# maniacs-ops/ringpop-go

Measured on AMD Instinct MI355X. Metric: simulated member-rounds/sec at 64k members, higher is better.
Workload: dtype u32; 1 GPU; config3_cascade: 65536 members, 655 killed at r=10; rounds 5-592 timed (steady state, kill, suspect wave; faulty wave from r>=35 in window); members=65536, live_member_rounds=38153303, parallelism=1 GPU

## Files before the change

### include/swimsim.h

```cpp
#ifndef SWIMSIM_H
#define SWIMSIM_H
#include <stddef.h>
#include <stdint.h>

#ifdef __cplusplus
extern "C" {
#endif

#define SWIMSIM_ABI_VERSION 12

enum {
    SWIMSIM_OK = 0,
    SWIMSIM_EINVAL = -1,
    SWIMSIM_ENOMEM = -2,
    SWIMSIM_EHIP = -3,
    SWIMSIM_ECAPACITY = -4,
    SWIMSIM_ERANGE = -5
};

enum { SWIMSIM_ALIVE = 0, SWIMSIM_SUSPECT = 1, SWIMSIM_FAULTY = 2, SWIMSIM_LEAVE = 3, SWIMSIM_TOMBSTONE = 4,
       SWIMSIM_UNKNOWN = 7 };
#define SWIMSIM_SOURCE_NONE (-1)

typedef struct swimsim_config {
// ... 14 lines not shown
    uint64_t message_pool_bytes;
    uint32_t observer_begin, observer_end;
    const struct swimsim_tuning *tuning;
} swimsim_config;

typedef struct swimsim_tuning {
    int32_t hot_slots;
    int32_t dense_slots;
    int32_t cs_async;
    int32_t cs_async_rows;
    int32_t cs_narrow_rows;
    int32_t cs_ref;
    int32_t fault_inject;
    int32_t defer_test;
    int32_t cs_defer;
} swimsim_tuning;

enum {
    SWIMSIM_EV_KILL = 1,
    SWIMSIM_EV_REVIVE = 2,
    SWIMSIM_EV_REINCARNATE = 3,
    SWIMSIM_EV_LEAVE = 4,
    SWIMSIM_EV_PARTITION = 5,
    SWIMSIM_EV_HEAL = 6,
    SWIMSIM_EV_REAP = 7,
    SWIMSIM_EV_CLOCK = 8
};
typedef struct swimsim_event { uint32_t round; uint32_t kind; int32_t a; int32_t b; } swimsim_event;

enum {
// ... 126 lines not shown
```

### ringpop-go_amd/csrc/swimsim_device.h

```cpp
#pragma once
#include <hip/hip_runtime.h>
#include <stdint.h>

namespace swimdev {

constexpr uint32_t ST_ALIVE = 0, ST_SUSPECT = 1, ST_FAULTY = 2, ST_LEAVE = 3, ST_TOMB = 4, ST_UNKNOWN = 7;
constexpr uint32_t SRC_NONE = 0xFFFFFFFFu;
constexpr uint32_t NO_DEADLINE = 0xFFFFFFFFu;
constexpr uint8_t DP_NONE = 0xFF;
constexpr uint32_t DE_NONE = 0xFFFFFFFFu;
__host__ __device__ inline uint32_t de_p(uint32_t x) { return x >> 24; }
__host__ __device__ inline uint32_t de_src(uint32_t x) { return (x & 0xFFFFFFu) == 0xFFFFFFu ? SRC_NONE : (x & 0xFFFFFFu); }
__host__ __device__ inline uint32_t de_x(uint32_t src, uint32_t p) { return (src & 0xFFFFFFu) | (p << 24); }

enum Counter {
    C_ROUNDS, C_PINGS, C_PINGS_OK, C_PINGREQS, C_HELPER_CALLS, C_HELPER_ERRORS, C_INCONCLUSIVE,
    C_SUSPECT_DECL, C_APPLIED, C_REFUTES, C_FULL_SYNCS, C_FULL_SYNCS_PINGREQ, C_RFS_DONE, C_RFS_OMITTED,
    C_TIMERS_FIRED, C_MSG_CHANGES, C_HEAL_ATTEMPTS, C_HEAL_FAILURES, C_NCOUNTERS,
    C_X_MERGED = C_NCOUNTERS, C_X_APPLIED, C_X_ISSUED, C_X_CS_ROWS, C_X_CS_DUP,
    C_X_MERGED_R, C_X_APPLIED_R, C_X_RISSUED, C_X_RCALLS, C_X_BUMPED, C_X_CS_ROWS_N, C_X_CSD_SCANNED,
    C_X_DENSE_RESP, C_X_DENSE_JOBS, C_X_JOBS_APPLIED, C_X_DENSE_HEAL,
    C_X_DEFER, C_X_DEFER_EQ, C_X_DEFER_NOROW, C_X_DEFER_REP, C_X_DEFER_UNDO,
    C_X_DEFER_REP_DIFF, C_X_DEFER_UNDO_DIFF, C_X_DEFER_FS, C_X_DEFER_UNDO_OVER, C_X_DEFER_CLEAN,
    C_X_ISSUE_SNAPS, C_X_LAZY_LATE, C_X_LAZY_MAT, C_NALL
};

constexpr int CTR_SHARDS = 64, CTR_STRIDE = 64;
static_assert(C_NALL <= CTR_STRIDE, "counter block too small");
constexpr uint32_t POOL_SHARDS = 64, POOL_CUR_STRIDE = 16;

enum ErrBits : uint32_t {
    E_POOL = 1, E_DENSE = 2, E_ECAP = 4, E_SHORT = 8, E_ITER = 16, E_COUNT = 32, E_XCAP = 64
};

struct MsgDesc {
    uint32_t off_lo, off_hi;
    uint32_t len;
    uint32_t kind;
};
// ... 58 lines not shown
    uint32_t *hmw;
    uint2 *hde;
    uint32_t *colx;
    uint32_t *hotnew;
    uint32_t *hot_cnt;
    uint32_t HP;
    int32_t *nhe;
    uint32_t *ucl, *uhk, *ucold, *ucnt;
    uint2 *ulog;
    uint32_t *ulog_cnt;
    uint32_t ulog_cap;
    uint32_t ulog_stride;
    uint32_t defer_test;
    uint32_t *ilen;
    int32_t *ilast;
};
constexpr uint32_t ULOG_CAP = 1024, ULOG_STRIDE = ULOG_CAP + 256;
constexpr uint32_t SRC_PEND = 0x7FFFFFFEu, SRC_CLAIM = 0x7FFFFFFDu;
constexpr uint32_t DIRTY_CARRIED = 2u;

__device__ __forceinline__ uint32_t hot_slot(const DS &d, uint32_t m) { return d.hidx ? d.hidx[m] : SRC_NONE; }

__host__ __device__ inline bool is_pingable(uint32_t st) { return st <= ST_SUSPECT; }

__device__ __forceinline__ uint32_t clock_of(const DS &d, uint32_t o, uint32_t r) { return r + (uint32_t)d.coff[o]; }

constexpr uint32_t RT_LOOKUP = 0, RT_COLD = 8191, RT_MAXSLOTS = 8128;
__host__ __device__ inline uint32_t rec_m(const uint4 &r) { return r.x & 0xFFFFFFu; }
__host__ __device__ inline uint32_t rec_st(const uint4 &r) { return (r.x >> 24) & 7u; }
__host__ __device__ inline uint32_t rec_e(const uint4 &r) { return r.y & 0xFFFFFFu; }
__host__ __device__ inline uint32_t rec_tag(const uint4 &r) { return (r.x >> 27) | ((r.y >> 24) << 5); }
__host__ __device__ inline uint32_t tag_of_slot(uint32_t hk) { return hk == SRC_NONE ? RT_COLD : hk + 1u; }
__host__ __device__ inline uint4 rec_make(uint32_t m, uint32_t st, uint32_t e, uint32_t src, uint32_t sinc, uint32_t tag) {
    return make_uint4(m | (st << 24) | (tag << 27), e | ((tag >> 5) << 24), src, sinc);
}
__host__ __device__ inline uint4 rec_retag(const uint4 &r, uint32_t tag) {
    return make_uint4((r.x & 0x07FFFFFFu) | (tag << 27), (r.y & 0xFFFFFFu) | ((tag >> 5) << 24), r.z, r.w);
}
__device__ __forceinline__ uint32_t rec_slot(const DS &d, const uint4 &r) {
    const uint32_t t = rec_tag(r);
    return t == RT_LOOKUP ? hot_slot(d, rec_m(r)) : t == RT_COLD ? SRC_NONE : t - 1u;
}
// ... 138 lines not shown
```

### ringpop-go_amd/csrc/swimsim_engine.hip

```cpp
#include "swimsim_kernels.hip"
#include "swimsim_xchg.hip"
#include "swimsim_census.hip"
#include "swimsim_route.hip"

#include <hipcub/hipcub.hpp>
#include <rccl/rccl.h>

#include <algorithm>
#include <cmath>
#include <condition_variable>
#include <cstdarg>
#include <cstdio>
#include <cstring>
#include <memory>
#include <mutex>
#include <string>
#include <thread>
#include <vector>

#include "../../include/swimsim.h"

using namespace swimdev;

namespace {
// ... 333 lines not shown
    size_t rt_bytes_cap = 0, rt_keys_cap = 0, rt_rows_cap = 0, rt_own_cap = 0, rt_exc_cap = 0, rt_cub_bytes = 0;
    std::vector<uint64_t> rt_rel;
    hipEvent_t rt_ev[2] = {nullptr, nullptr};
    int csr_mode = 1;
    CsrSet csr, csr2;
    size_t csr_sbw_words = 0;
    uint32_t csr_ecap = 4096, csr_rcap = 1024, csr_KP = 0;
    uint64_t csr_launches = 0;
    uint32_t csr_side_min = 4097;
    int fault_inject = 0;
    int defer_test = 0;
    int cs_defer = 1;
    uint32_t rounds_left = 0;
    uint32_t round_deferred = 0;
    bool cs_carried = false;
    bool cs_defer_log = false;
    uint64_t cs_skipped_rounds = 0, cs_carried_rows = 0, cs_forced = 0, cs_units_base[3] = {0, 0, 0};
    bool colx_stale = false;
    std::string err;

    int fail(int code, const char *fmt, ...) {
        char buf[512];
        va_list ap;
        va_start(ap, fmt);
        vsnprintf(buf, sizeof buf, fmt, ap);
        va_end(ap);
        err = buf;
        return code;
    }
};
// ... 1259 lines not shown
        return bail(SWIMSIM_EHIP);
    }
    const swimsim_tuning *tun = cfg->tuning;
    if (tun && tun->cs_async >= 0) h->cs_async = tun->cs_async != 0;
    if (tun && tun->cs_narrow_rows >= 0) h->cs_narrow_rows = (uint32_t)tun->cs_narrow_rows;
    if (tun && tun->cs_ref >= 0) h->csr_mode = tun->cs_ref;
    if (tun && tun->fault_inject > 0) h->fault_inject = tun->fault_inject;
    if (tun && tun->defer_test > 0) h->defer_test = tun->defer_test;
    if (tun && tun->cs_defer >= 0) h->cs_defer = tun->cs_defer;
    if (const char *v = getenv("SWIMSIM_CS_DEFER")) h->cs_defer = atoi(v);
    if (const char *v = getenv("SWIMSIM_CS_DEFER_LOG")) h->cs_defer_log = atoi(v) != 0;
    if (h->cs_defer < 0 || h->cs_defer > 2) {
        h->err = "swimsim_tuning.cs_defer is -1, 0, 1 or 2";
        return bail(SWIMSIM_EINVAL);
    }
    if (h->fault_inject & 32) h->csr_ecap = 24;
    if (h->fault_inject & 256) h->csr_side_min = 1024;
    if (const char *v = getenv("SWIMSIM_SYNC_SPIN")) h->sync_spin = atoi(v) != 0;
    if (const char *v = getenv("SWIMSIM_SIDE2"))
        if (atoi(v) == 0 && h->side2) { hipStreamDestroy(h->side2); h->side2 = nullptr; }
    DS &d = h->d;
    d.N = h->N; d.NP = h->NP; d.NL = h->NL; d.lo = h->lo;
    d.NB = h->NP / 64;
    d.NBW = (d.NB + 63) / 64;
    d.NBIT = ((h->NP / 32) + 3) & ~3u;
    d.W = h->W; d.pfactor = h->pfactor; d.K = h->K; d.maxjobs = h->maxjobs;
    d.to_susp = h->to_susp; d.to_faulty = h->to_faulty; d.to_tomb = h->to_tomb;
    d.seed = h->seed;
    const size_t rows = (size_t)h->NL * h->NP;
    int rc = 0;
// ... 14 lines not shown
        (rc = dalloc(h, &d.colx, d.NBIT, "divergent columns")) || (rc = dalloc(h, &d.ucl, h->N, "divergent column list")) ||
        (rc = dalloc(h, &d.uhk, h->N, "divergent column hot slots")) || (rc = dalloc(h, &d.ucold, h->N, "cold divergent columns")) ||
        (rc = dalloc(h, &d.ucnt, 2, "divergent column counts")))
        return bail(rc);
    hipMemset(d.nhe, 0, (size_t)h->NL * 4);
    hipMemset(d.coff, 0, (size_t)h->N * 4);
    h->coff.assign(h->N, 0);
    hipMemset(d.colx, 0xFF, (size_t)d.NBIT * 4);
    hipMemset(d.cpslot, 0xFF, (size_t)h->NL * 4);
    {
        uint32_t hp = std::min<uint32_t>(2048u, h->NP);
        if (tun && tun->hot_slots >= 0) hp = std::min<uint32_t>((uint32_t)tun->hot_slots, h->NP);
        hp = std::min<uint32_t>((hp + 63) & ~63u, RT_MAXSLOTS);
        d.hidx = nullptr; d.hlist = nullptr; d.hmw = nullptr; d.hde = nullptr; d.hotnew = nullptr; d.hot_cnt = nullptr;
        d.HP = 0;
        if (hp) {
            if ((rc = dalloc(h, &d.hidx, h->N, "hot index")) || (rc = dalloc(h, &d.hlist, hp, "hot list")) ||
                (rc = dalloc(h, &d.hmw, (size_t)h->NL * hp, "hot member words")) ||
                (rc = dalloc(h, &d.hde, (size_t)h->NL * hp, "hot dissemination cells")) ||
                (rc = dalloc(h, &d.hotnew, d.NBIT, "hot candidates")) || (rc = dalloc(h, &d.hot_cnt, 2, "hot count")))
                return bail(rc);
            d.HP = hp;
            hot_reset(h, false);
        }
    }
    {
        std::vector<uint32_t> aw((size_t)h->N * 6, 0u);
        for (uint32_t m = 0; m < h->N; m++) {
            uint8_t b[24] = {0};
            memcpy(b, h->addrs[m].data(), h->W);
            for (int w = 0; w < 6; w++)
                aw[(size_t)m * 6 + w] = (uint32_t)b[4 * w] | ((uint32_t)b[4 * w + 1] << 8) | ((uint32_t)b[4 * w + 2] << 16) |
                                        ((uint32_t)b[4 * w + 3] << 24);
        }
        uint32_t *dev = nullptr;
        if ((rc = dalloc(h, &dev, aw.size(), "address words"))) return bail(rc);
        if (hipMemcpy(dev, aw.data(), aw.size() * 4, hipMemcpyHostToDevice) != hipSuccess) return bail(SWIMSIM_EHIP);
// ... 1067 lines not shown
        }
    }
    if (n) *n = F_NFAM;
    return SWIMSIM_OK;
}

int swimsim_kernel_units(swimsim_t *h, const char **names, double *values, size_t cap, size_t *n) {
    if (!h) return SWIMSIM_EINVAL;
    uint64_t c[CTR_STRIDE];
    if (int rc = read_counters(h, c)) return rc;
    static const char *kn[] = {"cs_rows_wide", "cs_rows_narrow", "cs_dup_rows", "recv_merged", "recv_applied",
                               "recv_issued", "recv_calls", "resp_merged", "resp_applied", "resp_bumped", "issued",
                               "bitmap_words_per_row", "hot_slots", "dense_resp", "dense_jobs", "jobs_applied",
                               "dense_heal", "defer", "defer_eq", "defer_norow", "defer_rep", "defer_undo",
                               "defer_rep_diff", "defer_undo_diff", "defer_fs", "defer_undo_over", "defer_clean",
                               "issue_snaps", "lazy_late", "lazy_mat",
                               "cs_skipped_rounds", "cs_carried_rows", "cs_forced"};
    const int ki[] = {C_X_CS_ROWS, C_X_CS_ROWS_N, C_X_CS_DUP, C_X_MERGED, C_X_APPLIED, C_X_RISSUED, C_X_RCALLS,
                      C_X_MERGED_R, C_X_APPLIED_R, C_X_BUMPED, C_X_ISSUED, -1, -2, C_X_DENSE_RESP, C_X_DENSE_JOBS,
                      C_X_JOBS_APPLIED, C_X_DENSE_HEAL, C_X_DEFER, C_X_DEFER_EQ, C_X_DEFER_NOROW, C_X_DEFER_REP,
                      C_X_DEFER_UNDO, C_X_DEFER_REP_DIFF, C_X_DEFER_UNDO_DIFF, C_X_DEFER_FS, C_X_DEFER_UNDO_OVER,
                      C_X_DEFER_CLEAN, C_X_ISSUE_SNAPS, C_X_LAZY_LATE, C_X_LAZY_MAT,
                      -3, -4, -5};
    const uint64_t lazy_c[3] = {h->cs_skipped_rounds - h->cs_units_base[0], h->cs_carried_rows - h->cs_units_base[1],
                                h->cs_forced - h->cs_units_base[2]};
    static_assert(sizeof(kn) / sizeof(kn[0]) == sizeof(ki) / sizeof(ki[0]), "one counter per name");
    uint32_t hot = 0;
    if (h->d.hot_cnt) {
        HIPCHK(h, hipMemcpyAsync(&hot, h->d.hot_cnt, 4, hipMemcpyDeviceToHost, h->s));
        HIPCHK(h, stream_sync(h));
    }
    const size_t k = sizeof(ki) / sizeof(ki[0]);
    for (size_t i = 0; i < k && i < cap; i++) {
        if (names) names[i] = kn[i];
        if (values)
            values[i] = ki[i] == -1 ? (double)h->d.NBIT : ki[i] == -2 ? (double)hot : ki[i] <= -3 ? (double)lazy_c[-3 - ki[i]]
                                                                                : (double)(c[ki[i]] - h->fam_bytes_base[ki[i]]);
// ... 197 lines not shown
```

### ringpop-go_amd/csrc/swimsim_kernels.hip

```cpp
#include "swimsim_kernels.h"

namespace swimdev {

#define SWIM_DPP(old, src, ctrl, rm) ((uint32_t)__builtin_amdgcn_update_dpp((int)(old), (int)(src), (ctrl), (rm), 0xf, false))
template <typename Op>
__device__ __forceinline__ uint32_t dpp_scan(uint32_t x, uint32_t id, Op op) {
    x = op(x, SWIM_DPP(id, x, 0x111, 0xf));
    x = op(x, SWIM_DPP(id, x, 0x112, 0xf));
    x = op(x, SWIM_DPP(id, x, 0x114, 0xf));
    x = op(x, SWIM_DPP(id, x, 0x118, 0xf));
    x = op(x, SWIM_DPP(id, x, 0x142, 0xa));
    x = op(x, SWIM_DPP(id, x, 0x143, 0xc));
    return x;
}
__device__ __forceinline__ uint32_t dpp_scan_add(uint32_t x) { return dpp_scan(x, 0u, [](uint32_t a, uint32_t b) { return a + b; }); }
__device__ __forceinline__ uint32_t dpp_scan_umin(uint32_t x) {
    return dpp_scan(x, 0xFFFFFFFFu, [](uint32_t a, uint32_t b) { return min(a, b); });
}
__device__ __forceinline__ int32_t dpp_scan_imax(int32_t x) {
    return (int32_t)dpp_scan((uint32_t)x, 0x80000000u, [](uint32_t a, uint32_t b) { return (uint32_t)max((int32_t)a, (int32_t)b); });
}
__device__ __forceinline__ int32_t dpp_scan_imin(int32_t x) {
    return (int32_t)dpp_scan((uint32_t)x, 0x7FFFFFFFu, [](uint32_t a, uint32_t b) { return (uint32_t)min((int32_t)a, (int32_t)b); });
}
// ... 330 lines not shown
                merge_change_w(d, ol, o, m, cur[u], w[u] & 7u, w[u] >> 3, meta.x, meta.y, now_e, sched_r, acc);
        }
    }
}

__device__ __forceinline__ void merge_first(const DS &d, const MsgDesc &md, uint4 (&rec)[MB]) {
    const unsigned long long off = ((unsigned long long)md.off_hi << 32) | md.off_lo;
#pragma unroll
    for (int u = 0; u < MB; u++) {
        const uint32_t i = u * 64 + lane_id();
        rec[u] = md.kind == 0 && i < md.len ? d.pool[off + i] : make_uint4(0xFFFFFFFFu, 0, 0, 0);
    }
}
__device__ __forceinline__ void wave_merge_body(const DS &d, uint32_t ol, uint32_t o, const MsgDesc &md, uint32_t now_e,
                                                uint32_t sched_r, MAcc &acc, int dctr, const uint4 *pre0 = nullptr,
                                                uint32_t *ulog = nullptr, LazyCtx *lz = nullptr) {
    const uint32_t *rowp = d.mw + (size_t)ol * d.NP;
    const uint32_t *hrow = d.hmw + (size_t)ol * d.HP;
    if (md.kind == 0) {
        const unsigned long long off = ((unsigned long long)md.off_hi << 32) | md.off_lo;
        for (uint32_t base = 0; base < md.len; base += 64 * MB) {
            uint4 rec[MB];
            uint32_t cur[MB], hk[MB];
#pragma unroll
            for (int u = 0; u < MB; u++) {
                const uint32_t i = base + u * 64 + lane_id();
                rec[u] = pre0 && base == 0 ? pre0[u] : i < md.len ? d.pool[off + i] : make_uint4(0xFFFFFFFFu, 0, 0, 0);
            }
#pragma unroll
            for (int u = 0; u < MB; u++) hk[u] = rec[u].x != 0xFFFFFFFFu ? rec_slot(d, rec[u]) : SRC_NONE;
#pragma unroll
            for (int u = 0; u < MB; u++)
                cur[u] = rec[u].x == 0xFFFFFFFFu ? 0u : hk[u] != SRC_NONE ? hrow[hk[u]] : rowp[rec_m(rec[u])];
#pragma unroll
            for (int u = 0; u < MB; u++) {
                const int before = acc.napp;
                if (rec[u].x != 0xFFFFFFFFu)
                    merge_change_w(d, ol, o, rec_m(rec[u]), cur[u], rec_st(rec[u]), rec_e(rec[u]), rec[u].z, rec[u].w, now_e,
                                   sched_r, acc, hk[u]);
                if (ulog) {
                    const bool ap = acc.napp != before;
                    const unsigned long long b = __ballot(ap);
                    const uint32_t at = *ulog + (uint32_t)__popcll(b & lanemask_lt());
                    if (ap && at < d.ulog_stride) d.ulog[(size_t)ol * d.ulog_stride + at] = make_uint2(rec_m(rec[u]), cur[u]);
                    *ulog += (uint32_t)__popcll(b);
                }
            }
            if (ulog && lz && lz->pend && *ulog > d.ulog_cap) wave_lazy_late(d, ol, o, *lz, *ulog);
        }
    } else if (md.kind == 1) {
        if (ulog && lz && lz->pend) wave_lazy_late(d, ol, o, *lz, *ulog);
        wave_merge_dense(d, ol, o, md, now_e, sched_r, acc);
        if (dctr >= 0 && lane_id() == 0) ctr_add(d, dctr, 1ull);
        if (ulog) *ulog = d.ulog_cap + 1u;
    }
    __threadfence_block();
}
__device__ void wave_merge_msg(const DS &d, uint32_t ol, uint32_t o, const MsgDesc &md, uint32_t now_e, uint32_t sched_r,
                               int cset = 0, int dctr = -1) {
    MAcc acc;
    acc_begin(d, ol, acc);
    wave_merge_body(d, ol, o, md, now_e, sched_r, acc, dctr);
    wave_finalize(d, ol, acc, cset);
}
__device__ __forceinline__ void wave_merge_msg_pre(const DS &d, uint32_t ol, uint32_t o, const MsgDesc &md, uint32_t now_e,
                                                   uint32_t sched_r, int cset, RowPre &p, int dctr = -1,
                                                   const uint4 *pre0 = nullptr, bool logit = false,
                                                   LazyCtx *lz = nullptr) {
    MAcc acc;
    acc.tag = p.useq;
    wave_merge_body(d, ol, o, md, now_e, sched_r, acc, dctr, pre0, logit && d.ulog ? &p.ulog : nullptr, lz);
    wave_finalize_pre(d, ol, acc, cset, p);
}

__device__ __forceinline__ int2 wave_bump_body(const DS &d, uint32_t ol, const MsgDesc &md, int maxp) {
    if (md.kind != 0) return make_int2(0, 0);
    const unsigned long long off = ((unsigned long long)md.off_hi << 32) | md.off_lo;
    uint32_t *dx = (uint32_t *)(d.dent + (size_t)ol * d.NP);
    uint32_t *hx = (uint32_t *)(d.hde + (size_t)ol * d.HP);
    int del = 0, delnh = 0;
    for (uint32_t base = 0; base < md.len; base += 64 * MB) {
        uint32_t m[MB], x[MB], hk[MB];
#pragma unroll
        for (int u = 0; u < MB; u++) {
            const uint32_t i = base + u * 64 + lane_id();
            const uint2 xy = i < md.len ? *(const uint2 *)(d.pool + off + i) : make_uint2(0xFFFFFFFFu, 0u);
// ... 26 lines not shown
__device__ void wave_bump(const DS &d, uint32_t ol, const MsgDesc &md) {
    if (md.kind != 0) return;
    const int2 dd = wave_bump_body(d, ol, md, d.maxp[ol]);
    if (lane_id() == 0 && dd.x) d.dcnt[ol] -= dd.x;
    if (lane_id() == 0 && dd.y) d.nhe[ol] -= dd.y;
    __threadfence_block();
}
__device__ __forceinline__ void wave_bump_pre(const DS &d, uint32_t ol, const MsgDesc &md, RowPre &p) {
    if (md.kind != 0) return;
    const int2 dd = wave_bump_body(d, ol, md, p.maxp);
    if (dd.x) { p.dcnt -= dd.x; if (lane_id() == 0) d.dcnt[ol] = p.dcnt; }
    if (dd.y) { p.nhe -= dd.y; if (lane_id() == 0) d.nhe[ol] = p.nhe; }
    __threadfence_block();
}

__device__ __forceinline__ unsigned long long pool_alloc_lane0(const DS &d, uint32_t n) {
    const unsigned long long sub = d.pool_cap / POOL_SHARDS;
    const bool small = n <= sub / 256;
    for (uint32_t t = 0, s = wave_gid() % POOL_SHARDS; t < POOL_SHARDS; t++, s = (s + 1) % POOL_SHARDS) {
        unsigned long long *cur = d.pool_cur + (size_t)s * POOL_CUR_STRIDE;
        if (small) {
            const unsigned long long old = atomicAdd(cur, (unsigned long long)n);
            if (old + n <= sub) return s * sub + old;
            continue;
        }
        unsigned long long old = __hip_atomic_load(cur, __ATOMIC_RELAXED, __HIP_MEMORY_SCOPE_AGENT);
        while (old + n <= sub) {
            const unsigned long long seen = atomicCAS(cur, old, old + n);
            if (seen == old) return s * sub + old;
            old = seen;
// ... 5 lines not shown
__device__ __forceinline__ unsigned long long pool_alloc(const DS &d, uint32_t n) {
    unsigned long long off = 0;
    if (lane_id() == 0 && n) off = pool_alloc_lane0(d, n);
    return bcast64(off);
}

__device__ __forceinline__ uint32_t wscan_excl(uint32_t v, uint32_t &total) {
    const uint32_t x = dpp_scan_add(v);
    total = lane63(x);
    return x - v;
}

template <bool RECV>
__device__ __forceinline__ uint32_t wave_issue_body(const DS &d, uint32_t ol, uint32_t sender, uint32_t sinc, MsgDesc &out,
                                                    uint32_t cnt, int maxp, bool hotwalk, uint32_t nslots,
                                                    unsigned long long off, int &del_out, int &delnh_out) {
    const size_t rb = (size_t)ol * d.NP, hb = (size_t)ol * d.HP;
    uint32_t *bits = d.dbit + (size_t)ol * d.NBIT;
    uint32_t pos = 0;
    int del = 0, delnh = 0;
    if (hotwalk) {
        for (uint32_t base = 0; base < nslots; base += 64 * MB) {
            uint2 ce[MB];
            uint32_t wv[MB], m[MB];
#pragma unroll
            for (int u = 0; u < MB; u++) {
                const uint32_t k = base + u * 64 + lane_id();
                ce[u] = k < nslots ? d.hde[hb + k] : make_uint2(DE_NONE, 0);
                wv[u] = k < nslots ? d.hmw[hb + k] : 0u;
                m[u] = k < nslots ? d.hlist[k] : 0u;
            }
            bool keep[MB];
            uint32_t nk = 0;
#pragma unroll
            for (int u = 0; u < MB; u++) {
                const uint32_t src = de_src(ce[u].x);
                keep[u] = de_p(ce[u].x) != DP_NONE && !(RECV && src == sender && ce[u].y == sinc);
                nk += keep[u] ? 1u : 0u;
            }
            uint32_t tot;
            uint32_t at = pos + wscan_excl(nk, tot);
#pragma unroll
            for (int u = 0; u < MB; u++) {
                if (!keep[u]) continue;
                const uint32_t st = (wv[u] & 7u) == ST_UNKNOWN ? ST_TOMB : (wv[u] & 7u);
                if (at < cnt) d.pool[off + at] = rec_make(m[u], st, wv[u] >> 3, de_src(ce[u].x), ce[u].y, base + u * 64 + lane_id() + 1u);
                at++;
                if (RECV) {
                    const uint32_t k = base + u * 64 + lane_id();
                    uint32_t nx;
                    if ((int)(de_p(ce[u].x) + 1) >= maxp) {
                        nx = ce[u].x | 0xFF000000u;
                        atomicAnd(bits + (m[u] >> 5), ~(1u << (m[u] & 31)));
                        del++;
                    } else {
                        nx = ce[u].x + (1u << 24);
                    }
                    d.hde[hb + k].x = nx;
                }
            }
            pos += tot;
        }
    } else if ((uint64_t)cnt * 4u > d.NP) {
        const uint2 *dcell = d.dent + rb;
        const uint32_t *drow = d.mw + rb;
        for (uint32_t base = 0; base < d.NP; base += 64 * MB) {
            uint2 ce[MB];
            uint32_t wv[MB], hk[MB];
#pragma unroll
            for (int u = 0; u < MB; u++) {
                const uint32_t m = base + u * 64 + lane_id();
                const bool in = m < d.N;
                hk[u] = in && d.hidx ? d.hidx[m] : SRC_NONE;
                ce[u] = in ? dcell[m] : make_uint2(DE_NONE, 0);
                wv[u] = in ? drow[m] : 0u;
            }
// ... 126 lines not shown
            pos += tot;
        }
        if (RECV && (dlo | dhi)) {
            if (dlo & 0xFFFFFFFFull) atomicAnd(bits + q + 0, ~(uint32_t)dlo);
            if (dlo >> 32) atomicAnd(bits + q + 1, ~(uint32_t)(dlo >> 32));
            if (dhi & 0xFFFFFFFFull) atomicAnd(bits + q + 2, ~(uint32_t)dhi);
            if (dhi >> 32) atomicAnd(bits + q + 3, ~(uint32_t)(dhi >> 32));
        }
    }
    if (RECV) {
        del_out = wsum(del);
        delnh_out = wsum(delnh);
    } else if (pos != cnt && lane_id() == 0) {
        atomicOr(d.err, E_COUNT);
    }
    out.off_lo = (uint32_t)off;
    out.off_hi = (uint32_t)(off >> 32);
    out.len = min(pos, cnt);
    return out.len;
}

template <bool RECV>
__device__ uint32_t wave_issue_t(const DS &d, uint32_t ol, uint32_t sender, uint32_t sinc, MsgDesc &out) {
    const uint32_t cnt = (uint32_t)d.dcnt[ol];
    const int maxp = RECV ? d.maxp[ol] : 0;
    const bool hotwalk = d.hidx && d.nhe[ol] == 0;
    const uint32_t nslots = d.hidx ? d.hot_cnt[0] : 0u;
    out.kind = 0; out.len = 0; out.off_lo = out.off_hi = 0;
    if (cnt == 0) return 0;
    const unsigned long long off = pool_alloc(d, cnt);
    if (off == ~0ull) return 0;
    int del = 0, delnh = 0;
    const uint32_t n = wave_issue_body<RECV>(d, ol, sender, sinc, out, cnt, maxp, hotwalk, nslots, off, del, delnh);
    if (RECV) {
        if (lane_id() == 0 && del) d.dcnt[ol] -= del;
        if (lane_id() == 0 && delnh) d.nhe[ol] -= delnh;
    }
    __threadfence_block();
    return n;
}

__device__ void wave_issue(const DS &d, uint32_t ol, MsgDesc &out) { wave_issue_t<false>(d, ol, 0, 0, out); }

__device__ uint32_t wave_issue_recv(const DS &d, uint32_t ol, uint32_t sender, uint32_t sinc, MsgDesc &out) {
    return wave_issue_t<true>(d, ol, sender, sinc, out);
}

__device__ bool wave_snapshot(const DS &d, uint32_t ol, uint32_t o, MsgDesc &out) {
    uint32_t slot = 0;
    if (lane_id() == 0) slot = atomicAdd(d.dense_cur, 1u);
    slot = (uint32_t)__builtin_amdgcn_readlane((int)slot, 0);
    out.kind = 2; out.len = 0; out.off_lo = out.off_hi = 0;
    if (slot >= d.dense_cap) {
        if (lane_id() == 0) atomicOr(d.err, E_DENSE);
        return false;
    }
    const uint4 *src = (const uint4 *)(d.mw + (size_t)ol * d.NP);
// ... 396 lines not shown
}

__global__ void k_issue(DS d, int mode, const int32_t *tgt, const uint8_t *failed, MsgDesc *sdesc, uint32_t *sI,
                        uint32_t *sC, uint32_t *sS) {
    const uint32_t ol = wave_gid();
    if (ol >= d.NL) return;
    const uint32_t o = d.lo + ol;
    if ((mode == 0 && tgt[ol] < 0) || (mode == 1 && !failed[ol])) {
        if (sS && lane_id() == 0) sS[o] = SRC_NONE;
        return;
    }
    const uint32_t dirty = d.dirty[ol], cpslot = d.cpslot[ol], cs = d.cs[ol], selfw = d.mw[(size_t)ol * d.NP + o];
    const uint32_t clen = d.clen[ol];
    const int32_t clast = d.clast[ol];
    MsgDesc md;
    wave_issue(d, ol, md);
    uint32_t slot = SRC_NONE;
    if (sS && dirty && !d.ulog) {
        MsgDesc sn;
        if (wave_snapshot(d, ol, o, sn)) slot = sn.off_lo;
        if (lane_id() == 0) ctr_add(d, C_X_ISSUE_SNAPS, 1ull);
    } else if (sS && dirty) {
        slot = SRC_PEND;
        if (lane_id() == 0) { d.ilen[ol] = clen; d.ilast[ol] = clast; }
    } else if (sS) {
        slot = cpslot;
    }
    if (lane_id() == 0) {
        sdesc[o] = md;
        sI[o] = selfw >> 3;
        sC[o] = slot == SRC_NONE ? cs : 0u;
// ... 121 lines not shown
};

__global__ void k_pair_info(const DS d, const uint32_t *vals, uint32_t n, int phase, const MsgDesc *sdesc, const uint32_t *sI,
                            const uint32_t *sC, const uint32_t *sS, uint4 *pinfo) {
    const uint32_t i = blockIdx.x * blockDim.x + threadIdx.x;
    if (d.ulog_cnt && i < d.NL) d.ulog_cnt[i] = 0u;
    if (i >= n) return;
    const uint32_t v = vals[i], sender = phase == 0 ? v : v / d.K;
    if (sender >= d.N) return;
    const MsgDesc md = sdesc[sender];
    pinfo[2 * (size_t)i] = make_uint4(md.off_lo, md.off_hi, md.len, md.kind);
    pinfo[2 * (size_t)i + 1] = make_uint4(sI[sender], sC[sender], sS ? sS[sender] : SRC_NONE, v);
}

__device__ __forceinline__ void recv_one_pre(const DS &d, const RecvArgs &a, uint32_t j, const uint4 pi0, const uint4 pi1,
                                             uint32_t pair, uint32_t nslots, uint32_t now, RowPre &p, LazyCtx &lz) {
    const uint32_t ol = j - d.lo;
    const uint32_t v = pi1.w, sender = a.phase == 0 ? v : v / d.K, resp_idx = v;
    MsgDesc md;
    md.off_lo = pi0.x; md.off_hi = pi0.y; md.len = pi0.z; md.kind = pi0.w;
    const uint64_t bound = (uint64_t)(uint32_t)p.dcnt + md.len;
    const bool early = md.kind == 0 && bound > 0 && bound <= min(4096ull, d.pool_cap / POOL_SHARDS / 16);
    unsigned long long roff = 0;
    if (early && lane_id() == 0) roff = pool_alloc_lane0(d, (uint32_t)bound);
    wave_merge_msg_pre(d, ol, j, md, now, now, 0, p, -1, nullptr, true, &lz);
    MsgDesc resp;
    resp.kind = 0; resp.len = 0; resp.off_lo = resp.off_hi = 0;
    uint32_t kept = 0;
    const uint32_t cnt = (uint32_t)p.dcnt;
    if (cnt) {
        const unsigned long long off = early ? bcast64(roff) : pool_alloc(d, cnt);
        if (off != ~0ull) {
            int del = 0, delnh = 0;
            kept = wave_issue_body<true>(d, ol, sender, pi1.x, resp, cnt, p.maxp, d.hidx && p.nhe == 0, nslots, off, del,
                                         delnh);
            if (del) { p.dcnt -= del; if (lane_id() == 0) d.dcnt[ol] = p.dcnt; }
            if (delnh) { p.nhe -= delnh; if (lane_id() == 0) d.nhe[ol] = p.nhe; }
            __threadfence_block();
        }
    }
    if (lane_id() == 0) {
        ctr_add(d, C_X_RISSUED, (unsigned long long)kept);
        ctr_add(d, C_X_RCALLS, 1ull);
    }
    if (kept == 0) {
        const uint32_t scs = pi1.y;
        const uint32_t sslot = a.sS ? pi1.z : SRC_NONE;
        const bool rdirty = p.dirty != 0;
        const uint32_t rpend = rdirty ? SRC_NONE : p.cpslot;
        if (rdirty || rpend != SRC_NONE || sslot != SRC_NONE) {
            if (wave_snapshot(d, ol, j, resp) && lane_id() == 0) {
                if (rpend != SRC_NONE) d.dense_meta[resp.off_lo].w = rpend + 1u;
                else if (!rdirty) d.dense_cs[resp.off_lo] = p.cs;
                a.defer[atomicAdd(a.defer_cnt, 1u)] =
                    make_uint4(resp_idx | (rdirty ? 0x80000000u : 0u), resp.off_lo, sslot != SRC_NONE ? sslot : scs,
                               pair | (sslot != SRC_NONE ? 0x80000000u : 0u));
            }
            resp.kind = 2;
        } else if (p.cs != scs) {
            wave_snapshot(d, ol, j, resp);
            if (lane_id() == 0) {
                if (a.phase == 0) a.fsflag[pair] = 1;
                ctr_add(d, a.phase == 0 ? C_FULL_SYNCS : C_FULL_SYNCS_PINGREQ, 1ull);
            }
        }
    }
    if (lane_id() == 0) {
        a.rdesc[resp_idx] = resp;
        if (resp.kind != 2) ctr_add(d, C_MSG_CHANGES, (unsigned long long)resp.len);
        if (a.phase == 1) {
            ctr_add(d, C_HELPER_CALLS, 1ull);
            ctr_add(d, C_MSG_CHANGES, (unsigned long long)md.len);
        }
    }
}

constexpr int RECV_MIN_WAVES = 4;
__global__ void __launch_bounds__(256, RECV_MIN_WAVES) k_recv(DS d, RecvArgs a) {
    const uint32_t u = wave_gid();
    if (u >= a.nruns_max) return;
    const uint32_t key = a.ukeys[u];
    if (key >= d.N) return;
    const uint32_t n = a.counts[u], off = a.offs[u];
    RowPre p = row_pre(d, key - d.lo);
    const uint32_t now = wave_clock(d, key, a.r);
    const uint32_t nslots = d.hidx ? d.hot_cnt[0] : 0u;
    LazyCtx lz;
    lz.sS = a.sS; lz.sI = a.sI;
    lz.pend = a.sS && d.ulog && uni(a.sS[key]) == SRC_PEND;
    for (uint32_t w = 0; w < n; w++) {
        const uint32_t pair = off + w;
        recv_one_pre(d, a, key, a.pinfo[2 * (size_t)pair], a.pinfo[2 * (size_t)pair + 1], pair, nslots, now, p, lz);
    }
    if (d.ulog_cnt && lane_id() == 0) d.ulog_cnt[key - d.lo] = min(p.ulog, d.ulog_cap + 1u);
}

__global__ void k_colx_rebuild(DS d) {
    const uint32_t m = blockIdx.x * blockDim.x + threadIdx.x;
    bool diff = false;
    if (m < d.N) {
        const uint32_t w0 = d.mw[m];
        for (uint32_t ol = 1; ol < d.NL && !diff; ol++) diff = d.mw[(size_t)ol * d.NP + m] != w0;
    }
    const unsigned long long bits = __ballot(diff);
    const uint32_t w = (m & ~63u) >> 5;
    if (lane_id() == 0) {
        if (w < d.NBIT) d.colx[w] = (uint32_t)bits;
// ... 291 lines not shown
        fsflag[p] = 0;
        if (d.njobs[ol] < d.maxjobs) d.jobs[(size_t)ol * d.maxjobs + d.njobs[ol]++] = vals[p];
        else ctr_add(d, C_RFS_OMITTED, 1ull);
    }
}

__global__ void k_resp(DS d, const int32_t *tgt, const uint8_t *failed, const MsgDesc *sdesc, const MsgDesc *rdesc,
                       uint32_t r) {
    const uint32_t ol = wave_gid();
    if (ol >= d.NL) return;
    if (tgt[ol] < 0 || failed[ol]) return;
    const uint32_t o = d.lo + ol;
    RowPre p = row_pre(d, ol);
    const uint32_t now = wave_clock(d, o, r);
    const MsgDesc sd = sdesc[o], rd = rdesc[o];
    uint4 rec0[MB];
    merge_first(d, rd, rec0);
    wave_bump_pre(d, ol, sd, p);
    wave_merge_msg_pre(d, ol, o, rd, now, now, 1, p, C_X_DENSE_RESP, rec0);
    if (lane_id() == 0) {
        ctr_add(d, C_PINGS_OK, 1ull);
        if (sd.kind == 0) ctr_add(d, C_X_BUMPED, (unsigned long long)sd.len);
    }
}

__global__ void k_resolve(DS d, const int32_t *tgt, const uint8_t *failed, const uint32_t *H, const uint32_t *nh,
                          const MsgDesc *sdesc2, const MsgDesc *rdesc2, uint32_t r) {
    const uint32_t ol = wave_gid();
    if (ol >= d.NL || !failed[ol]) return;
    const uint32_t o = d.lo + ol, K = d.K;
    const uint32_t now = wave_clock(d, o, r);
    uint32_t errs = 0;
    for (uint32_t q = 0; q < nh[ol]; q++) {
        const uint32_t h = H[(size_t)ol * K + q];
        if (!reach(d, o, h)) {
            errs++;
            wave_bump(d, ol, sdesc2[o]);
// ... 386 lines not shown
```

### ringpop-go_amd/swimsim/__init__.py

```python
from __future__ import annotations

import ctypes as C
import os
from dataclasses import dataclass

import numpy as np

_HERE = os.path.dirname(os.path.abspath(__file__))
LIB_PATH = os.path.join(_HERE, "libswimsim.so")

ALIVE, SUSPECT, FAULTY, LEAVE, TOMBSTONE, UNKNOWN = 0, 1, 2, 3, 4, 7
STATUS_NAMES = {ALIVE: "alive", SUSPECT: "suspect", FAULTY: "faulty", LEAVE: "leave", TOMBSTONE: "tombstone"}
SOURCE_NONE = -1
EV_KILL, EV_REVIVE, EV_REINCARNATE, EV_LEAVE, EV_PARTITION, EV_HEAL, EV_REAP = 1, 2, 3, 4, 5, 6, 7
EV_CLOCK = 8
COUNTER_NAMES = [
    "rounds", "pings", "pings_ok", "pingreqs", "helper_calls", "helper_errors", "inconclusive",
    "suspect_decl", "applied", "refutes", "full_syncs", "full_syncs_pingreq", "rfs_done",
    "rfs_omitted", "timers_fired", "msg_changes", "heal_attempts", "heal_failures",
]
T0_MS = 1_500_000_000_000
CENSUS_LIVE, CENSUS_ALL = 0, 1
CENSUS_WHO = {"live": CENSUS_LIVE, "all": CENSUS_ALL}
ROUTE_N_REPLICAS = 16
# ... 8 lines not shown
class Config(C.Structure):
    _fields_ = [
        ("num_members", C.c_uint32), ("device", C.c_uint32), ("t0_ms", C.c_int64),
        ("protocol_period_ms", C.c_uint32), ("suspect_timeout_ms", C.c_uint32), ("faulty_timeout_ms", C.c_uint32),
        ("tombstone_timeout_ms", C.c_uint32), ("ping_request_size", C.c_uint32),
        ("max_reverse_full_sync_jobs", C.c_uint32), ("p_factor", C.c_uint32), ("seed", C.c_uint64),
        ("addresses", C.c_char_p), ("addr_stride", C.c_uint32), ("max_rounds", C.c_uint32),
        ("message_pool_bytes", C.c_uint64), ("observer_begin", C.c_uint32), ("observer_end", C.c_uint32),
        ("tuning", C.c_void_p),
    ]


class Tuning(C.Structure):
    _fields_ = [("hot_slots", C.c_int32), ("dense_slots", C.c_int32), ("cs_async", C.c_int32),
                ("cs_async_rows", C.c_int32), ("cs_narrow_rows", C.c_int32), ("cs_ref", C.c_int32),
                ("fault_inject", C.c_int32), ("defer_test", C.c_int32), ("cs_defer", C.c_int32)]


def make_tuning(tuning):
    if not tuning:
        return None
    t = Tuning(*([-1] * len(Tuning._fields_)))
    for k, v in tuning.items():
        if k not in dict(Tuning._fields_):
            raise ValueError(f"unknown tuning field {k}")
        setattr(t, k, int(v))
    return t


class Event(C.Structure):
    _fields_ = [("round", C.c_uint32), ("kind", C.c_uint32), ("a", C.c_int32), ("b", C.c_int32)]
# ... 1020 lines not shown
```

Baseline: 97.93 million member-rounds/s.

## Skip echoing merged hot records in responses and bump only sent slots

Adds an echo_skip mode, on by default. During receive merges, a per-wave shared-memory mask records the hot slots whose incoming state already equals the local state. The response builder then skips writing those records to the pool while still counting them logically. Separately, the ping sender records a per-row bitmask of the hot slots it actually sent, and the response-apply kernel bumps piggyback counters only for those slots instead of walking the sent message. This cuts pool writes and bump work, at the cost of extra mask memory, atomics and semantics that must stay equivalent to the original protocol.

```diff
diff --git a/include/swimsim.h b/include/swimsim.h
--- a/include/swimsim.h
+++ b/include/swimsim.h
@@ -7,7 +7,7 @@
 extern "C" {
 #endif
 
-#define SWIMSIM_ABI_VERSION 12
+#define SWIMSIM_ABI_VERSION 13
 
 enum {
     SWIMSIM_OK = 0,
@@ -52,6 +52,7 @@
     int32_t fault_inject;
     int32_t defer_test;
     int32_t cs_defer;
+    int32_t echo_skip;
 } swimsim_tuning;
 
 enum {
diff --git a/ringpop-go_amd/csrc/swimsim_device.h b/ringpop-go_amd/csrc/swimsim_device.h
--- a/ringpop-go_amd/csrc/swimsim_device.h
+++ b/ringpop-go_amd/csrc/swimsim_device.h
@@ -22,7 +22,8 @@
     C_X_DENSE_RESP, C_X_DENSE_JOBS, C_X_JOBS_APPLIED, C_X_DENSE_HEAL,
     C_X_DEFER, C_X_DEFER_EQ, C_X_DEFER_NOROW, C_X_DEFER_REP, C_X_DEFER_UNDO,
     C_X_DEFER_REP_DIFF, C_X_DEFER_UNDO_DIFF, C_X_DEFER_FS, C_X_DEFER_UNDO_OVER, C_X_DEFER_CLEAN,
-    C_X_ISSUE_SNAPS, C_X_LAZY_LATE, C_X_LAZY_MAT, C_NALL
+    C_X_ISSUE_SNAPS, C_X_LAZY_LATE, C_X_LAZY_MAT,
+    C_X_RESP_ECHO, C_X_BUMP_SLOT, C_NALL
 };
 
 constexpr int CTR_SHARDS = 64, CTR_STRIDE = 64;
@@ -111,7 +112,12 @@
     uint32_t defer_test;
     uint32_t *ilen;
     int32_t *ilast;
-};
+    unsigned long long *smask;
+    uint32_t *smask_n;
+    uint32_t echo_skip;
+};
+constexpr uint32_t ECHO_RESP = 1u, ECHO_BUMP = 2u;
+
 constexpr uint32_t ULOG_CAP = 1024, ULOG_STRIDE = ULOG_CAP + 256;
 constexpr uint32_t SRC_PEND = 0x7FFFFFFEu, SRC_CLAIM = 0x7FFFFFFDu;
 constexpr uint32_t DIRTY_CARRIED = 2u;
@@ -123,6 +129,8 @@
 __device__ __forceinline__ uint32_t clock_of(const DS &d, uint32_t o, uint32_t r) { return r + (uint32_t)d.coff[o]; }
 
 constexpr uint32_t RT_LOOKUP = 0, RT_COLD = 8191, RT_MAXSLOTS = 8128;
+constexpr uint32_t ECHO_WORDS = 256;
+static_assert(ECHO_WORDS * 32 >= RT_COLD && RT_MAXSLOTS <= ECHO_WORDS * 32, "the echo mask covers every tag");
 __host__ __device__ inline uint32_t rec_m(const uint4 &r) { return r.x & 0xFFFFFFu; }
 __host__ __device__ inline uint32_t rec_st(const uint4 &r) { return (r.x >> 24) & 7u; }
 __host__ __device__ inline uint32_t rec_e(const uint4 &r) { return r.y & 0xFFFFFFu; }
diff --git a/ringpop-go_amd/csrc/swimsim_engine.hip b/ringpop-go_amd/csrc/swimsim_engine.hip
--- a/ringpop-go_amd/csrc/swimsim_engine.hip
+++ b/ringpop-go_amd/csrc/swimsim_engine.hip
@@ -371,6 +371,7 @@
     uint32_t rounds_left = 0;
     uint32_t round_deferred = 0;
     bool cs_carried = false;
+    int echo_skip = 1;
     bool cs_defer_log = false;
     uint64_t cs_skipped_rounds = 0, cs_carried_rows = 0, cs_forced = 0, cs_units_base[3] = {0, 0, 0};
     bool colx_stale = false;
@@ -1660,6 +1661,12 @@
         h->err = "swimsim_tuning.cs_defer is -1, 0, 1 or 2";
         return bail(SWIMSIM_EINVAL);
     }
+    if (tun && tun->echo_skip >= 0) h->echo_skip = tun->echo_skip;
+    if (const char *v = getenv("SWIMSIM_ECHO_SKIP")) h->echo_skip = atoi(v);
+    if (h->echo_skip < 0 || h->echo_skip > 3) {
+        h->err = "swimsim_tuning.echo_skip is -1, 0, 1, 2 or 3";
+        return bail(SWIMSIM_EINVAL);
+    }
     if (h->fault_inject & 32) h->csr_ecap = 24;
     if (h->fault_inject & 256) h->csr_side_min = 1024;
     if (const char *v = getenv("SWIMSIM_SYNC_SPIN")) h->sync_spin = atoi(v) != 0;
@@ -1704,6 +1711,7 @@
         hp = std::min<uint32_t>((hp + 63) & ~63u, RT_MAXSLOTS);
         d.hidx = nullptr; d.hlist = nullptr; d.hmw = nullptr; d.hde = nullptr; d.hotnew = nullptr; d.hot_cnt = nullptr;
         d.HP = 0;
+        d.smask = nullptr; d.smask_n = nullptr; d.echo_skip = 0;
         if (hp) {
             if ((rc = dalloc(h, &d.hidx, h->N, "hot index")) || (rc = dalloc(h, &d.hlist, hp, "hot list")) ||
                 (rc = dalloc(h, &d.hmw, (size_t)h->NL * hp, "hot member words")) ||
@@ -1711,6 +1719,14 @@
                 (rc = dalloc(h, &d.hotnew, d.NBIT, "hot candidates")) || (rc = dalloc(h, &d.hot_cnt, 2, "hot count")))
                 return bail(rc);
             d.HP = hp;
+            d.echo_skip = h->echo_skip == 1 ? (ECHO_RESP | ECHO_BUMP) : h->echo_skip == 2 ? ECHO_RESP
+                          : h->echo_skip == 3 ? ECHO_BUMP : 0u;
+            if (d.echo_skip & ECHO_BUMP) {
+                if ((rc = dalloc(h, &d.smask, (size_t)h->NL * (hp / 64), "sent-slot masks")) ||
+                    (rc = dalloc(h, &d.smask_n, h->NL, "sent-slot counts")))
+                    return bail(rc);
+                hipMemset(d.smask_n, 0, (size_t)h->NL * 4);
+            }
             hot_reset(h, false);
         }
     }
@@ -2808,13 +2824,13 @@
                                "bitmap_words_per_row", "hot_slots", "dense_resp", "dense_jobs", "jobs_applied",
                                "dense_heal", "defer", "defer_eq", "defer_norow", "defer_rep", "defer_undo",
                                "defer_rep_diff", "defer_undo_diff", "defer_fs", "defer_undo_over", "defer_clean",
-                               "issue_snaps", "lazy_late", "lazy_mat",
+                               "issue_snaps", "lazy_late", "lazy_mat", "resp_echo", "bump_slot_rows",
                                "cs_skipped_rounds", "cs_carried_rows", "cs_forced"};
     const int ki[] = {C_X_CS_ROWS, C_X_CS_ROWS_N, C_X_CS_DUP, C_X_MERGED, C_X_APPLIED, C_X_RISSUED, C_X_RCALLS,
                       C_X_MERGED_R, C_X_APPLIED_R, C_X_BUMPED, C_X_ISSUED, -1, -2, C_X_DENSE_RESP, C_X_DENSE_JOBS,
                       C_X_JOBS_APPLIED, C_X_DENSE_HEAL, C_X_DEFER, C_X_DEFER_EQ, C_X_DEFER_NOROW, C_X_DEFER_REP,
                       C_X_DEFER_UNDO, C_X_DEFER_REP_DIFF, C_X_DEFER_UNDO_DIFF, C_X_DEFER_FS, C_X_DEFER_UNDO_OVER,
-                      C_X_DEFER_CLEAN, C_X_ISSUE_SNAPS, C_X_LAZY_LATE, C_X_LAZY_MAT,
+                      C_X_DEFER_CLEAN, C_X_ISSUE_SNAPS, C_X_LAZY_LATE, C_X_LAZY_MAT, C_X_RESP_ECHO, C_X_BUMP_SLOT,
                       -3, -4, -5};
     const uint64_t lazy_c[3] = {h->cs_skipped_rounds - h->cs_units_base[0], h->cs_carried_rows - h->cs_units_base[1],
                                 h->cs_forced - h->cs_units_base[2]};
diff --git a/ringpop-go_amd/csrc/swimsim_kernels.hip b/ringpop-go_amd/csrc/swimsim_kernels.hip
--- a/ringpop-go_amd/csrc/swimsim_kernels.hip
+++ b/ringpop-go_amd/csrc/swimsim_kernels.hip
@@ -368,7 +368,8 @@
 }
 __device__ __forceinline__ void wave_merge_body(const DS &d, uint32_t ol, uint32_t o, const MsgDesc &md, uint32_t now_e,
                                                 uint32_t sched_r, MAcc &acc, int dctr, const uint4 *pre0 = nullptr,
-                                                uint32_t *ulog = nullptr, LazyCtx *lz = nullptr) {
+                                                uint32_t *ulog = nullptr, LazyCtx *lz = nullptr,
+                                                uint32_t *emask = nullptr, uint32_t sender = SRC_NONE) {
     const uint32_t *rowp = d.mw + (size_t)ol * d.NP;
     const uint32_t *hrow = d.hmw + (size_t)ol * d.HP;
     if (md.kind == 0) {
@@ -388,10 +389,16 @@
                 cur[u] = rec[u].x == 0xFFFFFFFFu ? 0u : hk[u] != SRC_NONE ? hrow[hk[u]] : rowp[rec_m(rec[u])];
 #pragma unroll
             for (int u = 0; u < MB; u++) {
-                const int before = acc.napp;
+                const int before = acc.napp, rbefore = acc.nref;
                 if (rec[u].x != 0xFFFFFFFFu)
                     merge_change_w(d, ol, o, rec_m(rec[u]), cur[u], rec_st(rec[u]), rec_e(rec[u]), rec[u].z, rec[u].w, now_e,
                                    sched_r, acc, hk[u]);
+                if (emask && rec[u].x != 0xFFFFFFFFu && hk[u] != SRC_NONE && rec_st(rec[u]) <= ST_LEAVE &&
+                    rec_m(rec[u]) != sender) {
+                    const bool same = acc.napp != before ? acc.nref == rbefore
+                                                         : cur[u] == ((rec_e(rec[u]) << 3) | rec_st(rec[u]));
+                    if (same) atomicOr(emask + (hk[u] >> 5), 1u << (hk[u] & 31));
+                }
                 if (ulog) {
                     const bool ap = acc.napp != before;
                     const unsigned long long b = __ballot(ap);
@@ -420,10 +427,11 @@
 __device__ __forceinline__ void wave_merge_msg_pre(const DS &d, uint32_t ol, uint32_t o, const MsgDesc &md, uint32_t now_e,
                                                    uint32_t sched_r, int cset, RowPre &p, int dctr = -1,
                                                    const uint4 *pre0 = nullptr, bool logit = false,
-                                                   LazyCtx *lz = nullptr) {
+                                                   LazyCtx *lz = nullptr, uint32_t *emask = nullptr,
+                                                   uint32_t sender = SRC_NONE) {
     MAcc acc;
     acc.tag = p.useq;
-    wave_merge_body(d, ol, o, md, now_e, sched_r, acc, dctr, pre0, logit && d.ulog ? &p.ulog : nullptr, lz);
+    wave_merge_body(d, ol, o, md, now_e, sched_r, acc, dctr, pre0, logit && d.ulog ? &p.ulog : nullptr, lz, emask, sender);
     wave_finalize_pre(d, ol, acc, cset, p);
 }
 
@@ -480,6 +488,55 @@
     __threadfence_block();
 }
 
+struct SlotPre {
+    uint32_t x[MB];
+    unsigned long long w[MB];
+};
+__device__ __forceinline__ void slot_first(const DS &d, uint32_t ol, SlotPre &sp) {
+    const uint32_t *hx = (const uint32_t *)(d.hde + (size_t)ol * d.HP);
+    const unsigned long long *sm = d.smask + (size_t)ol * (d.HP / 64);
+#pragma unroll
+    for (int u = 0; u < MB; u++) {
+        const uint32_t k = u * 64 + lane_id();
+        sp.x[u] = k < d.HP ? hx[(size_t)k * 2] : DE_NONE;
+        sp.w[u] = (uint32_t)u * 64 < d.HP ? sm[u] : 0ull;
+    }
+}
+__device__ __forceinline__ void wave_bump_slots_pre(const DS &d, uint32_t ol, uint32_t sn, const SlotPre &sp, RowPre &p) {
+    uint32_t *hx = (uint32_t *)(d.hde + (size_t)ol * d.HP);
+    const unsigned long long *sm = d.smask + (size_t)ol * (d.HP / 64);
+    int del = 0;
+    for (uint32_t base = 0; base < sn; base += 64 * MB) {
+        uint32_t x[MB];
+        unsigned long long w[MB];
+#pragma unroll
+        for (int u = 0; u < MB; u++) {
+            const uint32_t k = base + u * 64 + lane_id();
+            x[u] = base == 0 ? sp.x[u] : k < sn ? hx[(size_t)k * 2] : DE_NONE;
+            w[u] = base == 0 ? sp.w[u] : base + u * 64 < sn ? sm[(base >> 6) + u] : 0ull;
+        }
+#pragma unroll
+        for (int u = 0; u < MB; u++) {
+            const uint32_t k = base + u * 64 + lane_id();
+            const uint32_t pc = de_p(x[u]);
+            if (k >= sn || !((w[u] >> lane_id()) & 1ull) || pc == DP_NONE) continue;
+            uint32_t nx;
+            if ((int)(pc + 1) >= p.maxp) {
+                nx = x[u] | 0xFF000000u;
+                const uint32_t m = d.hlist[k];
+                atomicAnd(&d.dbit[(size_t)ol * d.NBIT + (m >> 5)], ~(1u << (m & 31)));
+                del++;
+            } else {
+                nx = x[u] + (1u << 24);
+            }
+            hx[(size_t)k * 2] = nx;
+        }
+    }
+    del = wsum(del);
+    if (del) { p.dcnt -= del; if (lane_id() == 0) d.dcnt[ol] = p.dcnt; }
+    __threadfence_block();
+}
+
 __device__ __forceinline__ unsigned long long pool_alloc_lane0(const DS &d, uint32_t n) {
     const unsigned long long sub = d.pool_cap / POOL_SHARDS;
     const bool small = n <= sub / 256;
@@ -515,21 +572,24 @@
 template <bool RECV>
 __device__ __forceinline__ uint32_t wave_issue_body(const DS &d, uint32_t ol, uint32_t sender, uint32_t sinc, MsgDesc &out,
                                                     uint32_t cnt, int maxp, bool hotwalk, uint32_t nslots,
-                                                    unsigned long long off, int &del_out, int &delnh_out) {
+                                                    unsigned long long off, int &del_out, int &delnh_out,
+                                                    const uint32_t *emask = nullptr, unsigned long long *smask = nullptr) {
     const size_t rb = (size_t)ol * d.NP, hb = (size_t)ol * d.HP;
     uint32_t *bits = d.dbit + (size_t)ol * d.NBIT;
-    uint32_t pos = 0;
+    uint32_t pos = 0, logical = 0;
     int del = 0, delnh = 0;
     if (hotwalk) {
         for (uint32_t base = 0; base < nslots; base += 64 * MB) {
             uint2 ce[MB];
             uint32_t wv[MB], m[MB];
+            bool echo[MB];
 #pragma unroll
             for (int u = 0; u < MB; u++) {
                 const uint32_t k = base + u * 64 + lane_id();
+                echo[u] = RECV && emask && k < nslots && ((emask[k >> 5] >> (k & 31)) & 1u);
                 ce[u] = k < nslots ? d.hde[hb + k] : make_uint2(DE_NONE, 0);
-                wv[u] = k < nslots ? d.hmw[hb + k] : 0u;
-                m[u] = k < nslots ? d.hlist[k] : 0u;
+                wv[u] = k < nslots && !echo[u] ? d.hmw[hb + k] : 0u;
+                m[u] = k < nslots && !echo[u] ? d.hlist[k] : 0u;
             }
             bool keep[MB];
             uint32_t nk = 0;
@@ -537,22 +597,32 @@
             for (int u = 0; u < MB; u++) {
                 const uint32_t src = de_src(ce[u].x);
                 keep[u] = de_p(ce[u].x) != DP_NONE && !(RECV && src == sender && ce[u].y == sinc);
-                nk += keep[u] ? 1u : 0u;
+                nk += keep[u] ? (echo[u] ? 1u : 0x10001u) : 0u;
+            }
+            if (!RECV && smask) {
+#pragma unroll
+                for (int u = 0; u < MB; u++) {
+                    const unsigned long long b = __ballot(keep[u]);
+                    if (lane_id() == 0 && base + u * 64 < nslots) smask[(base >> 6) + u] = b;
+                }
             }
             uint32_t tot;
-            uint32_t at = pos + wscan_excl(nk, tot);
+            uint32_t at = pos + (wscan_excl(nk, tot) >> 16);
 #pragma unroll
             for (int u = 0; u < MB; u++) {
                 if (!keep[u]) continue;
-                const uint32_t st = (wv[u] & 7u) == ST_UNKNOWN ? ST_TOMB : (wv[u] & 7u);
-                if (at < cnt) d.pool[off + at] = rec_make(m[u], st, wv[u] >> 3, de_src(ce[u].x), ce[u].y, base + u * 64 + lane_id() + 1u);
-                at++;
+                if (!echo[u]) {
+                    const uint32_t st = (wv[u] & 7u) == ST_UNKNOWN ? ST_TOMB : (wv[u] & 7u);
+                    if (at < cnt) d.pool[off + at] = rec_make(m[u], st, wv[u] >> 3, de_src(ce[u].x), ce[u].y, base + u * 64 + lane_id() + 1u);
+                    at++;
+                }
                 if (RECV) {
                     const uint32_t k = base + u * 64 + lane_id();
                     uint32_t nx;
                     if ((int)(de_p(ce[u].x) + 1) >= maxp) {
                         nx = ce[u].x | 0xFF000000u;
-                        atomicAnd(bits + (m[u] >> 5), ~(1u << (m[u] & 31)));
+                        const uint32_t mm = echo[u] ? d.hlist[k] : m[u];
+                        atomicAnd(bits + (mm >> 5), ~(1u << (mm & 31)));
                         del++;
                     } else {
                         nx = ce[u].x + (1u << 24);
@@ -560,7 +630,8 @@
                     d.hde[hb + k].x = nx;
                 }
             }
-            pos += tot;
+            pos += tot >> 16;
+            logical += tot & 0xFFFFu;
         }
     } else if ((uint64_t)cnt * 4u > d.NP) {
         const uint2 *dcell = d.dent + rb;
@@ -717,24 +788,26 @@
     } else if (pos != cnt && lane_id() == 0) {
         atomicOr(d.err, E_COUNT);
     }
+    if (!hotwalk) logical = pos;
     out.off_lo = (uint32_t)off;
     out.off_hi = (uint32_t)(off >> 32);
     out.len = min(pos, cnt);
-    return out.len;
+    return min(logical, cnt);
 }
 
 template <bool RECV>
-__device__ uint32_t wave_issue_t(const DS &d, uint32_t ol, uint32_t sender, uint32_t sinc, MsgDesc &out) {
+__device__ uint32_t wave_issue_t(const DS &d, uint32_t ol, uint32_t sender, uint32_t sinc, MsgDesc &out, bool sent = false) {
     const uint32_t cnt = (uint32_t)d.dcnt[ol];
     const int maxp = RECV ? d.maxp[ol] : 0;
     const bool hotwalk = d.hidx && d.nhe[ol] == 0;
     const uint32_t nslots = d.hidx ? d.hot_cnt[0] : 0u;
     out.kind = 0; out.len = 0; out.off_lo = out.off_hi = 0;
-    if (cnt == 0) return 0;
-    const unsigned long long off = pool_alloc(d, cnt);
+    const unsigned long long off = cnt ? pool_alloc(d, cnt) : ~0ull;
+    if (sent && lane_id() == 0) d.smask_n[ol] = hotwalk && off != ~0ull ? nslots : 0u;
     if (off == ~0ull) return 0;
     int del = 0, delnh = 0;
-    const uint32_t n = wave_issue_body<RECV>(d, ol, sender, sinc, out, cnt, maxp, hotwalk, nslots, off, del, delnh);
+    const uint32_t n = wave_issue_body<RECV>(d, ol, sender, sinc, out, cnt, maxp, hotwalk, nslots, off, del, delnh, nullptr,
+                                             sent ? d.smask + (size_t)ol * (d.HP / 64) : nullptr);
     if (RECV) {
         if (lane_id() == 0 && del) d.dcnt[ol] -= del;
         if (lane_id() == 0 && delnh) d.nhe[ol] -= delnh;
@@ -743,7 +816,9 @@
     return n;
 }
 
-__device__ void wave_issue(const DS &d, uint32_t ol, MsgDesc &out) { wave_issue_t<false>(d, ol, 0, 0, out); }
+__device__ void wave_issue(const DS &d, uint32_t ol, MsgDesc &out, bool sent = false) {
+    wave_issue_t<false>(d, ol, 0, 0, out, sent);
+}
 
 __device__ uint32_t wave_issue_recv(const DS &d, uint32_t ol, uint32_t sender, uint32_t sinc, MsgDesc &out) {
     return wave_issue_t<true>(d, ol, sender, sinc, out);
@@ -1170,7 +1245,7 @@
     const uint32_t clen = d.clen[ol];
     const int32_t clast = d.clast[ol];
     MsgDesc md;
-    wave_issue(d, ol, md);
+    wave_issue(d, ol, md, mode == 0 && (d.echo_skip & ECHO_BUMP));
     uint32_t slot = SRC_NONE;
     if (sS && dirty && !d.ulog) {
         MsgDesc sn;
@@ -1322,7 +1397,8 @@
 }
 
 __device__ __forceinline__ void recv_one_pre(const DS &d, const RecvArgs &a, uint32_t j, const uint4 pi0, const uint4 pi1,
-                                             uint32_t pair, uint32_t nslots, uint32_t now, RowPre &p, LazyCtx &lz) {
+                                             uint32_t pair, uint32_t nslots, uint32_t now, RowPre &p, LazyCtx &lz,
+                                             uint32_t *emask) {
     const uint32_t ol = j - d.lo;
     const uint32_t v = pi1.w, sender = a.phase == 0 ? v : v / d.K, resp_idx = v;
     MsgDesc md;
@@ -1331,7 +1407,12 @@
     const bool early = md.kind == 0 && bound > 0 && bound <= min(4096ull, d.pool_cap / POOL_SHARDS / 16);
     unsigned long long roff = 0;
     if (early && lane_id() == 0) roff = pool_alloc_lane0(d, (uint32_t)bound);
-    wave_merge_msg_pre(d, ol, j, md, now, now, 0, p, -1, nullptr, true, &lz);
+    if (p.nhe != 0) emask = nullptr;
+    if (emask) {
+        for (uint32_t i = lane_id(); i < (nslots + 31) / 32; i += 64) emask[i] = 0u;
+        __builtin_amdgcn_fence(__ATOMIC_RELEASE, "wavefront");
+    }
+    wave_merge_msg_pre(d, ol, j, md, now, now, 0, p, -1, nullptr, true, &lz, emask, sender);
     MsgDesc resp;
     resp.kind = 0; resp.len = 0; resp.off_lo = resp.off_hi = 0;
     uint32_t kept = 0;
@@ -1341,7 +1422,7 @@
         if (off != ~0ull) {
             int del = 0, delnh = 0;
             kept = wave_issue_body<true>(d, ol, sender, pi1.x, resp, cnt, p.maxp, d.hidx && p.nhe == 0, nslots, off, del,
-                                         delnh);
+                                         delnh, emask);
             if (del) { p.dcnt -= del; if (lane_id() == 0) d.dcnt[ol] = p.dcnt; }
             if (delnh) { p.nhe -= delnh; if (lane_id() == 0) d.nhe[ol] = p.nhe; }
             __threadfence_block();
@@ -1350,6 +1431,7 @@
     if (lane_id() == 0) {
         ctr_add(d, C_X_RISSUED, (unsigned long long)kept);
         ctr_add(d, C_X_RCALLS, 1ull);
+        if (kept != resp.len) ctr_add(d, C_X_RESP_ECHO, (unsigned long long)(kept - resp.len));
     }
     if (kept == 0) {
         const uint32_t scs = pi1.y;
@@ -1373,9 +1455,10 @@
             }
         }
     }
+    const uint32_t msg_changes = resp.kind == 0 ? kept : resp.len;
     if (lane_id() == 0) {
         a.rdesc[resp_idx] = resp;
-        if (resp.kind != 2) ctr_add(d, C_MSG_CHANGES, (unsigned long long)resp.len);
+        if (resp.kind != 2) ctr_add(d, C_MSG_CHANGES, (unsigned long long)msg_changes);
         if (a.phase == 1) {
             ctr_add(d, C_HELPER_CALLS, 1ull);
             ctr_add(d, C_MSG_CHANGES, (unsigned long long)md.len);
@@ -1396,9 +1479,11 @@
     LazyCtx lz;
     lz.sS = a.sS; lz.sI = a.sI;
     lz.pend = a.sS && d.ulog && uni(a.sS[key]) == SRC_PEND;
+    __shared__ uint32_t echo_s[256 / 64][ECHO_WORDS];
+    uint32_t *emask = d.hidx && (d.echo_skip & ECHO_RESP) ? echo_s[threadIdx.x >> 6] : nullptr;
     for (uint32_t w = 0; w < n; w++) {
         const uint32_t pair = off + w;
-        recv_one_pre(d, a, key, a.pinfo[2 * (size_t)pair], a.pinfo[2 * (size_t)pair + 1], pair, nslots, now, p, lz);
+        recv_one_pre(d, a, key, a.pinfo[2 * (size_t)pair], a.pinfo[2 * (size_t)pair + 1], pair, nslots, now, p, lz, emask);
     }
     if (d.ulog_cnt && lane_id() == 0) d.ulog_cnt[key - d.lo] = min(p.ulog, d.ulog_cap + 1u);
 }
@@ -1720,13 +1805,19 @@
     RowPre p = row_pre(d, ol);
     const uint32_t now = wave_clock(d, o, r);
     const MsgDesc sd = sdesc[o], rd = rdesc[o];
+    const bool bslot = d.smask && (d.echo_skip & ECHO_BUMP);
+    const uint32_t sn = bslot ? uni(d.smask_n[ol]) : 0u;
+    SlotPre sp;
+    if (bslot) slot_first(d, ol, sp);
     uint4 rec0[MB];
     merge_first(d, rd, rec0);
-    wave_bump_pre(d, ol, sd, p);
+    if (sn) wave_bump_slots_pre(d, ol, sn, sp, p);
+    else wave_bump_pre(d, ol, sd, p);
     wave_merge_msg_pre(d, ol, o, rd, now, now, 1, p, C_X_DENSE_RESP, rec0);
     if (lane_id() == 0) {
         ctr_add(d, C_PINGS_OK, 1ull);
         if (sd.kind == 0) ctr_add(d, C_X_BUMPED, (unsigned long long)sd.len);
+        if (sn) ctr_add(d, C_X_BUMP_SLOT, 1ull);
     }
 }
 
diff --git a/ringpop-go_amd/swimsim/__init__.py b/ringpop-go_amd/swimsim/__init__.py
--- a/ringpop-go_amd/swimsim/__init__.py
+++ b/ringpop-go_amd/swimsim/__init__.py
@@ -46,7 +46,8 @@
 class Tuning(C.Structure):
     _fields_ = [("hot_slots", C.c_int32), ("dense_slots", C.c_int32), ("cs_async", C.c_int32),
                 ("cs_async_rows", C.c_int32), ("cs_narrow_rows", C.c_int32), ("cs_ref", C.c_int32),
-                ("fault_inject", C.c_int32), ("defer_test", C.c_int32), ("cs_defer", C.c_int32)]
+                ("fault_inject", C.c_int32), ("defer_test", C.c_int32), ("cs_defer", C.c_int32),
+                ("echo_skip", C.c_int32)]
 
 
 def make_tuning(tuning):
```

Result: no change. 98.47 million member-rounds/s, median of 3 (+0.6%).
